# RolandFaure/Hairsplitter

Measured on AMD Instinct MI355X. Metric: aligned read-bp/sec through call_variants+separate_reads, higher is better.
Workload: dtype u8

## Files before the change

hairsplitter_amd/csrc/hs_kernels.hip:

```cpp
#include <hip/hip_runtime.h>
#include <stdint.h>
#include "hs_device.h"
#include "hs_rh8.h"

namespace hsdev {

static __device__ __forceinline__ int lane_id() { return (int)(threadIdx.x & 63u); }
static __device__ __forceinline__ int wave_id() { return __builtin_amdgcn_readfirstlane((int)(threadIdx.x >> 6)); }

static __device__ __forceinline__ unsigned long long wave_max_u64(unsigned long long v) {
#pragma unroll
    for (int d = 32; d >= 1; d >>= 1) {
        unsigned long long o = __shfl_xor(v, d, 64);
        v = o > v ? o : v;
    }
    return v;
}
static __device__ __forceinline__ int wave_scan_incl(int v) {
    v += __builtin_amdgcn_update_dpp(0, v, 0x111, 0xf, 0xf, false);
    v += __builtin_amdgcn_update_dpp(0, v, 0x112, 0xf, 0xf, false);
    v += __builtin_amdgcn_update_dpp(0, v, 0x114, 0xf, 0xf, false);
    v += __builtin_amdgcn_update_dpp(0, v, 0x118, 0xf, 0xf, false);
    v += __builtin_amdgcn_update_dpp(0, v, 0x142, 0xa, 0xf, false);
    v += __builtin_amdgcn_update_dpp(0, v, 0x143, 0xc, 0xf, false);
// ... 114 lines not shown
    const int rd = rec_read[r];
    const int64_t roff = read_off[rd];
    const int rlen = (int)(read_off[rd + 1] - roff);
    const int pos = rec_pos[r];
    const bool fwd = rec_strand[r] != 0;
    const int64_t cig0 = rec_cig_off[r], cig1 = rec_cig_off[r + 1];
    const int n_chunks = (int)((cig1 - cig0 + 63) >> 6);
    const int32_t* __restrict__ cs = chunk_start + 4 * rec_chunk_off[r];
    uint8_t* __restrict__ out = pile + pile_off[r];
    const uint8_t* __restrict__ ctgp = contig_seq + coff;
    const uint8_t* __restrict__ rdp = read_seq + roff;
    const unsigned long long lt_mask = (1ull << lane) - 1ull;
    const int rd_xor = fwd ? 0 : -1, rd_add = fwd ? 0 : rlen, rd_cmpl = fwd ? 0 : 3;

    int klo = 0, khi = n_chunks - 1;
    while (klo < khi) { const int mid = (klo + khi + 1) >> 1; if (cs[4 * mid] <= e_first) klo = mid; else khi = mid - 1; }

    int p1 = 2, p2 = 1;
    int nerr = 0, nlen = 0;
    for (int k = klo; k < n_chunks; ++k) {
        const int ev_base = cs[4 * k + 0];
        if (ev_base >= e1) break;
        const int t_cur = cs[4 * k + 1], q_cur = cs[4 * k + 2];
        const int64_t oi = cig0 + ((int64_t)k << 6) + lane;
        const bool in_range = oi < cig1;
        const uint32_t op = in_range ? cigar[oi] : 0xFu;
        const int code = in_range ? (int)(op & 15u) : 15;
        const OpAdv a = op_advances(op, in_range);
        const int ev_inc = wave_scan_incl(a.ev), rd_inc = wave_scan_incl(a.rd), rf_inc = wave_scan_incl(a.rf);
        const int ev_ex = ev_inc - a.ev;
        const int chunk_ev = __builtin_amdgcn_readlane(ev_inc, 63);
        const bool nz = a.ev > 0;
        const unsigned long long nzmask = __ballot(nz);
        wave_lds_sync();
        const bool isM = code == 0 || code == 7 || code == 8;
        s_op[wv][lane] = make_int4(ev_ex, t_cur + rd_inc - a.rd, q_cur + rf_inc - a.rf, (isM ? 1 : 0) | (code == 2 ? 3 : 0));
        if (nz) s_nzlane[wv][__popcll(nzmask & lt_mask)] = (uint8_t)lane;
        const int lo_el = e_first > ev_base ? e_first - ev_base : 0;
        const int hi_el = (e1 - ev_base) < chunk_ev ? (e1 - ev_base) : chunk_ev;
        const int lo_commit = e0 - ev_base;
        const unsigned span_commit = hi_el > lo_commit ? (unsigned)(hi_el - lo_commit) : 0u;

        uint8_t* const flags = &s_flag[wv][0][0];
        for (int eb = lo_el; eb < hi_el; eb += 64 * PU) {
#pragma unroll
            for (int z = 0; z < PU / 4; ++z) reinterpret_cast<uint32_t*>(flags)[lane + 64 * z] = 0u;
            wave_lds_sync();
            {
                const int rel = ev_ex - eb;
                if (nz && (unsigned)rel < (unsigned)(64 * PU)) flags[rel] = 1;
            }
            wave_lds_sync();
            int before = __popcll(__ballot(nz && ev_ex < eb));
            int q_[PU], c_[PU], cref_[PU];
            bool act_[PU], wr_[PU], jm_[PU];
#pragma unroll
            for (int u = 0; u < PU; ++u) {
                const int w0 = eb + 64 * u;
                const int own = (int)flags[64 * u + lane];
                const unsigned long long fm = __ballot(own != 0);
                const int e = w0 + lane;
                const int rank = (before - 1 + own + (int)__builtin_amdgcn_mbcnt_hi((uint32_t)(fm >> 32), __builtin_amdgcn_mbcnt_lo((uint32_t)fm, 0u))) & 63;
                before += __popcll(fm);
                const int4 od = s_op[wv][s_nzlane[wv][rank]];
                const int off = e - od.x;
                const bool refc = (od.w & 1) != 0, jD = (od.w & 2) != 0;
                const int t = od.y + off;
                const int q = od.z + (refc ? off : 0);
                act_[u] = (unsigned)(e - lo_commit) < span_commit && (unsigned)q < (unsigned)L;
                wr_[u] = refc; jm_[u] = od.w == 1; q_[u] = q;
                const int tt = clamp_i32(t, rlen - 1);
                const int bb = (int)rdp[(unsigned)((tt ^ rd_xor) + rd_add)];
                cref_[u] = (int)ctgp[(unsigned)clamp_i32(q, L - 1)];
                c_[u] = jD ? 4 : (bb ^ rd_cmpl);
            }
#pragma unroll
            for (int u = 0; u < PU; ++u) {
                const int w0 = eb + 64 * u;
                if (w0 >= hi_el) break;
                const int c = c_[u];
                const int cu1 = wave_shr1(c, p1);
                const int cu2 = wave_shr1(cu1, p2);
                nlen += __popcll(__ballot(act_[u]));
                nerr += __popcll(__ballot(act_[u] && !(jm_[u] && c == cref_[u])));
                if (act_[u] && wr_[u]) out[(unsigned)(q_[u] - pos)] = (uint8_t)(33 + 5 * cu2 + cu1 + 25 * c);
                const int nv = (hi_el - w0) < 64 ? (hi_el - w0) : 64;
                const int last = __builtin_amdgcn_readlane(c, nv - 1);
                const int last2 = nv >= 2 ? __builtin_amdgcn_readlane(c, nv - 2) : p1;
                p2 = last2; p1 = last;
            }
        }
    }
    if (lane == 0 && nlen > 0) {
        atomicAdd(&rec_stats[4 * r + 1], nerr);
        atomicAdd(&rec_stats[4 * r + 2], nlen);
    }
}

typedef uint32_t __attribute__((aligned(1))) u32_unaligned;
typedef uint16_t __attribute__((aligned(1))) u16_unaligned;
typedef uint32_t u32x4_unaligned __attribute__((ext_vector_type(4), aligned(1)));
static __device__ __forceinline__ uint32_t opaque(uint32_t x) { asm("" : "+v"(x)); return x; }
static __device__ __forceinline__ uint32_t bytes_ff(uint32_t x01) { return opaque(x01 << 8) - x01; }
static __device__ __forceinline__ uint32_t byte_sum(uint32_t x, uint32_t acc) { return __builtin_amdgcn_sad_u8(x, 0u, acc); }
static __device__ __forceinline__ uint32_t low_bytes(int n) { return n >= 4 ? 0xffffffffu : ((1u << (8 * n)) - 1u); }

#include "hs_kernels_runs.inc"

__global__ __launch_bounds__(256) void k_pileup_flagged_records(
    const uint8_t* __restrict__ contig_seq, const int64_t* __restrict__ contig_off,
    const uint8_t* __restrict__ read_seq, const int64_t* __restrict__ read_off,
    const int32_t* __restrict__ rec_read, const int32_t* __restrict__ rec_contig,
    const int32_t* __restrict__ rec_pos, const uint8_t* __restrict__ rec_strand,
    const int64_t* __restrict__ rec_cig_off, const uint32_t* __restrict__ cigar,
    const int64_t* __restrict__ pile_off, const int64_t* __restrict__ rec_chunk_off,
    const int32_t* __restrict__ chunk_start, int n_rec, int ev_per_task, uint8_t* __restrict__ pile, int32_t* __restrict__ rec_stats) {
    __shared__ PileupLds lds;
    const int lane = lane_id();
    const int wv = wave_id();
    const int n_waves = (int)gridDim.x * 4;
    for (int base = ((int)blockIdx.x * 4 + wv) * 64; base < n_rec; base += n_waves * 64) {
        const int rr = base + lane;
        bool flagged = false;
        if (rr < n_rec && rec_chunk_off[rr + 1] > rec_chunk_off[rr]) flagged = (chunk_start[4 * rec_chunk_off[rr] + 3] & 1) != 0;
        unsigned long long m = __ballot(flagged);
        while (m) {
            const int r = base + __builtin_ctzll(m);
            m &= m - 1ull;
            const int n_ev = rec_stats[4 * r + 3];
            for (int e0 = 0; e0 < n_ev; e0 += ev_per_task)
                pileup_task_per_event(lds, lane, wv, r, e0, ev_per_task, contig_seq, contig_off, read_seq, read_off, rec_read, rec_contig, rec_pos,
                                      rec_strand, rec_cig_off, cigar, pile_off, rec_chunk_off, chunk_start, pile, rec_stats);
        }
    }
}

#define HS_NBINS 125
#define HS_LIST_CAP 512
#ifndef HS_K2_INFLIGHT
#define HS_K2_INFLIGHT 16
#endif
template <int CB, bool FULL>
static __device__ __forceinline__ void column_stats_tail(const uint32_t* __restrict__ hw, int tid, int lane, int64_t g, int64_t total,
                                                         hs_colstat_dev* __restrict__ stats, int min_second, int32_t* __restrict__ sel_count,
                                                         int64_t* __restrict__ sel_gpos, int32_t* __restrict__ sel_depth, int sel_cap,
                                                         int64_t g_lo = 0, int64_t g_hi = 0x7fffffffffffffffll, int32_t* __restrict__ sel_ent = nullptr) {
    constexpr int PER_WORD = 4 / CB;
    constexpr int NWORDS = (HS_NBINS + PER_WORD - 1) / PER_WORD;
    int k0 = 0, k1 = 0, k2 = 0, k3 = 0;
    int c0 = 0, c1 = 0, c2 = 0, c3 = 0, c4 = 0;
    int depth = 0;
    if (!FULL) {
        if (g < total) {
            typedef unsigned short us2 __attribute__((ext_vector_type(2)));
            us2 m0a = {0, 0}, m1a = {0, 0}, m0b = {0, 0}, m1b = {0, 0};
#pragma unroll 4
            for (int w = 0; w < NWORDS; ++w) {
                const uint32_t word = hw[w * 256 + tid];
                us2 va, vb;
                if (CB == 1) {
                    depth = (int)__builtin_amdgcn_sad_u8(word, 0u, (uint32_t)depth);
                    va = __builtin_bit_cast(us2, word & 0x00ff00ffu);
                    vb = __builtin_bit_cast(us2, __builtin_amdgcn_perm(0u, word, 0x0c030c01u));
                } else {
                    depth += (int)(word & 0xffffu) + (int)(word >> 16);
                    va = __builtin_bit_cast(us2, word);
                    vb = us2{0, 0};
                }
                const us2 la = __builtin_elementwise_min(va, m0a);
                m1a = __builtin_elementwise_max(m1a, la);
                m0a = __builtin_elementwise_max(m0a, va);
                if (CB == 1) {
                    const us2 lb = __builtin_elementwise_min(vb, m0b);
                    m1b = __builtin_elementwise_max(m1b, lb);
                    m0b = __builtin_elementwise_max(m0b, vb);
                }
            }
            const int tops[8] = {m0a.x, m1a.x, m0a.y, m1a.y, m0b.x, m1b.x, m0b.y, m1b.y};
#pragma unroll
            for (int f = 0; f < 8; ++f) {
                const int v = tops[f];
                const int lo2 = v < c0 ? v : c0;
                c1 = c1 > lo2 ? c1 : lo2;
                c0 = c0 > v ? c0 : v;
            }
        }
        c2 = depth > c0 + c1 ? 1 : 0;
    } else if (g < total) {
        for (int w = 0; w < NWORDS; ++w) {
            const uint32_t word = hw[w * 256 + tid];
            if (word == 0u) continue;
#pragma unroll
            for (int f = 0; f < PER_WORD; ++f) {
                const int v = (int)((word >> (8 * CB * f)) & (CB == 1 ? 0xFFu : 0xFFFFu));
                if (v == 0) continue;
                depth += v;
                if (v > c4) {
                    const int key = w * PER_WORD + f + 33;
                    if (v > c0) { c4 = c3; c3 = c2; k3 = k2; c2 = c1; k2 = k1; c1 = c0; k1 = k0; c0 = v; k0 = key; }
                    else if (v > c1) { c4 = c3; c3 = c2; k3 = k2; c2 = c1; k2 = k1; c1 = v; k1 = key; }
                    else if (v > c2) { c4 = c3; c3 = c2; k3 = k2; c2 = v; k2 = key; }
                    else if (v > c3) { c4 = c3; c3 = v; k3 = key; }
                    else c4 = v;
                }
            }
        }
        uint4 o;
        o.x = (uint32_t)k0 | ((uint32_t)k1 << 8) | ((uint32_t)k2 << 16) | ((uint32_t)k3 << 24);
        o.y = (uint32_t)c0 | ((uint32_t)c1 << 16);
        o.z = (uint32_t)c2 | ((uint32_t)c3 << 16);
        o.w = (uint32_t)c4 | ((uint32_t)(depth > 65535 ? 65535 : depth) << 16);
        reinterpret_cast<uint4*>(stats)[g] = o;
    }
    if (sel_count) {
        __shared__ int s_wc[4], s_we[4];
        const bool sel = g < total && g >= g_lo && g < g_hi && (c1 > min_second || (c1 == min_second && c2 == 0));
        const unsigned long long m = __ballot(sel);
        const int wv = tid >> 6;
        if (lane == 0) s_wc[wv] = __popcll(m);
        if (sel_ent) { const int we = wave_sum_i32(sel ? depth : 0); if (lane == 0) s_we[wv] = we; }
        __syncthreads();
        int base = 0;
        for (int w = 0; w < wv; ++w) base += s_wc[w];
        const int64_t tile0 = (int64_t)blockIdx.x * 256;
        if (sel) {
            const int64_t slot = tile0 + base + __popcll(m & ((1ull << lane) - 1ull));
            sel_gpos[slot] = g; sel_depth[slot] = depth;
        }
        if (tid == 0) { sel_count[blockIdx.x] = s_wc[0] + s_wc[1] + s_wc[2] + s_wc[3]; if (sel_ent) sel_ent[blockIdx.x] = s_we[0] + s_we[1] + s_we[2] + s_we[3]; }
    }
}

__global__ __launch_bounds__(256) void k_selection_compact(const int32_t* __restrict__ tile_cnt, const int64_t* __restrict__ tile_base,
                                                          const int64_t* __restrict__ scratch_gpos, const int32_t* __restrict__ scratch_depth,
                                                          int64_t n_tiles, int32_t* __restrict__ out_count, int64_t* __restrict__ out_gpos,
                                                          int32_t* __restrict__ out_depth, int out_cap) {
    const int64_t t = blockIdx.x;
    const int tid = (int)threadIdx.x;
    if (t == 0 && tid == 0) *out_count = (int32_t)tile_base[n_tiles];
    if (tid < tile_cnt[t]) {
        const int64_t o = tile_base[t] + tid;
        if (o < out_cap) { out_gpos[o] = scratch_gpos[t * 256 + tid]; out_depth[o] = scratch_depth[t * 256 + tid]; }
    }
}

template <int CB, bool FULL, bool PAD>
__global__ __launch_bounds__(256) void k_column_stats_tiled(
    const uint8_t* __restrict__ pile, const int64_t* __restrict__ tile_off, const int4* __restrict__ tile_ent, int64_t total,
    hs_colstat_dev* __restrict__ stats, int min_second, int32_t* __restrict__ sel_count, int64_t* __restrict__ sel_gpos,
    int32_t* __restrict__ sel_depth, int sel_cap, int64_t tile0 ,
    int64_t g_lo, int64_t g_hi, int32_t* __restrict__ sel_ent) {
    constexpr int PER_WORD = 4 / CB;
    constexpr int NWORDS = (HS_NBINS + PER_WORD - 1) / PER_WORD;
    __shared__ __attribute__((aligned(16))) uint32_t hw[NWORDS * 256];
    const int tid = (int)threadIdx.x;
    const int lane = tid & 63;
    const int64_t tile = tile0 + (int64_t)blockIdx.x;
    const int64_t g = tile * 256 + tid;
#pragma unroll
    for (int w4 = 0; w4 < NWORDS; w4 += 4) {
        const int w = w4 + (lane >> 4);
        if (w < NWORDS) *reinterpret_cast<uint4*>(&hw[w * 256 + (tid & ~63) + (lane & 15) * 4]) = make_uint4(0u, 0u, 0u, 0u);
    }
    char* const my_col = reinterpret_cast<char*>(hw) + tid * 4;
    auto bump = [&](unsigned code, bool valid) {
        if (valid) {
            const unsigned inc = 1u << ((code & (unsigned)(PER_WORD - 1)) * (unsigned)(8 * CB));
            uint32_t* at = reinterpret_cast<uint32_t*>(my_col + ((code & ~(unsigned)(PER_WORD - 1)) << (CB == 1 ? 8 : 9)));
            __hip_atomic_fetch_add(at, inc, __ATOMIC_RELAXED, __HIP_MEMORY_SCOPE_WORKGROUP);
        }
    };
    const int64_t e0 = tile_off[tile], e1 = tile_off[tile + 1];
    for (int64_t i0 = e0; i0 < e1; i0 += 64) {
        const int nrec = (e1 - i0) < 64 ? (int)(e1 - i0) : 64;
        const int4 held = tile_ent[i0 + (lane < nrec ? lane : nrec - 1)];
        auto step = [&](int i, auto n_const) {
            constexpr int NU = decltype(n_const)::value;
            unsigned code[NU]; bool in_[NU];
#pragma unroll
            for (int u = 0; u < NU; ++u) {
                const int j = i + u;
                const int first = __builtin_amdgcn_readlane(held.x, j), len = __builtin_amdgcn_readlane(held.y, j);
                const uint32_t plo = (uint32_t)__builtin_amdgcn_readlane(held.z, j), phi = (uint32_t)__builtin_amdgcn_readlane(held.w, j);
                const uint8_t* __restrict__ base = pile + (int64_t)(((uint64_t)phi << 32) | plo);
                const bool in = (unsigned)(tid - first) < (unsigned)len;
                if (PAD) code[u] = (unsigned)base[tid] - 33u;
                else {
                    const unsigned off = (unsigned)(in ? tid : (first < 0 ? 0 : first));
                    code[u] = (unsigned)base[off] - 33u;
                }
                in_[u] = in;
            }
#pragma unroll
            for (int u = 0; u < NU; ++u) bump(code[u], in_[u] && code[u] < (unsigned)HS_NBINS);
        };
        int i = 0;
        for (; i + HS_K2_INFLIGHT <= nrec; i += HS_K2_INFLIGHT) step(i, std::integral_constant<int, HS_K2_INFLIGHT>());
        for (; i + 4 <= nrec; i += 4) step(i, std::integral_constant<int, 4>());
        for (; i < nrec; ++i) step(i, std::integral_constant<int, 1>());
    }
    column_stats_tail<CB, FULL>(hw, tid, lane, g, total, stats, min_second, sel_count, sel_gpos, sel_depth, sel_cap, g_lo, g_hi, sel_ent);
}

template <bool TOP >
static __device__ __forceinline__ void column_stats_tiled_dw_body(
    const uint8_t* __restrict__ pile, const int64_t* __restrict__ tile_off, const int4* __restrict__ tile_ent, int64_t total, int min_second,
    int32_t* __restrict__ sel_count, int64_t* __restrict__ sel_gpos, int32_t* __restrict__ sel_depth, int64_t tile0, int64_t g_lo, int64_t g_hi,
    int32_t* __restrict__ sel_ent, uint2* __restrict__ sel_info) {
    constexpr int NWORDS = (HS_NBINS + 3) / 4;
    static_assert(NWORDS == 32, "the second pass splits 32 counter words over four wavefronts");
    __shared__ __attribute__((aligned(16))) uint32_t hw[NWORDS * 256];
    __shared__ unsigned long long s_b[4];
    __shared__ int s_e[4];
    __shared__ uint8_t s_item[TOP ? 256 : 4];
    __shared__ uint32_t s_part[TOP ? 4 : 1][4][64];
    const int tid = (int)threadIdx.x;
    const int lane = tid & 63, wv = wave_id();
    const int64_t tile = tile0 + (int64_t)blockIdx.x;
#pragma unroll
    for (int x = 0; x < NWORDS * 256 / (256 * 4); ++x) reinterpret_cast<uint4*>(hw)[x * 256 + tid] = make_uint4(0u, 0u, 0u, 0u);
    __syncthreads();
    char* const my_cols = reinterpret_cast<char*>(hw) + lane * 4;
    auto bump = [&](unsigned code, bool valid, int k) {
        if (valid) {
            const unsigned inc = 1u << ((code & 3u) * 8u);
            uint32_t* at = reinterpret_cast<uint32_t*>(my_cols + 256 * k + ((code & ~3u) << 8));
#if defined(HS_K2_ABL) && HS_K2_ABL == 1
            asm volatile("" :: "v"(at), "v"(inc));
#else
            __hip_atomic_fetch_add(at, inc, __ATOMIC_RELAXED, __HIP_MEMORY_SCOPE_WORKGROUP);
#endif
        }
    };
    const int64_t e0 = tile_off[tile], e1 = tile_off[tile + 1];
    for (int64_t i0 = e0; i0 < e1; i0 += 64) {
        const int nrec = (e1 - i0) < 64 ? (int)(e1 - i0) : 64;
        const int4 held = tile_ent[i0 + (lane < nrec ? lane : nrec - 1)];
        auto step = [&](int j, auto n_const) {
            constexpr int NU = decltype(n_const)::value;
            uint32_t v[NU]; int first[NU], len[NU];
#pragma unroll
            for (int u = 0; u < NU; ++u) {
                const int jj = j + 4 * u;
                first[u] = __builtin_amdgcn_readlane(held.x, jj); len[u] = __builtin_amdgcn_readlane(held.y, jj);
                const uint32_t plo = (uint32_t)__builtin_amdgcn_readlane(held.z, jj), phi = (uint32_t)__builtin_amdgcn_readlane(held.w, jj);
                const uint8_t* __restrict__ base = pile + (int64_t)(((uint64_t)phi << 32) | plo);
#if defined(HS_K2_ABL) && HS_K2_ABL == 2
                v[u] = 0x41424344u + (uint32_t)lane + (uint32_t)(reinterpret_cast<uintptr_t>(base) & 3u);
#else
                v[u] = *reinterpret_cast<const u32_unaligned*>(base + 4 * lane);
#endif
            }
#pragma unroll
            for (int u = 0; u < NU; ++u) {
                if (first[u] == 0 && len[u] == 256) {
#pragma unroll
                    for (int k = 0; k < 4; ++k) { const unsigned code = ((v[u] >> (8 * k)) & 255u) - 33u; bump(code, code < (unsigned)HS_NBINS, k); }
                } else {
#pragma unroll
                    for (int k = 0; k < 4; ++k) {
                        const unsigned code = ((v[u] >> (8 * k)) & 255u) - 33u;
                        bump(code, (unsigned)(4 * lane + k - first[u]) < (unsigned)len[u] && code < (unsigned)HS_NBINS, k);
                    }
                }
            }
        };
        int j = wv;
        for (; j + 4 * 7 < nrec; j += 4 * 8) step(j, std::integral_constant<int, 8>());
        for (; j + 4 * 1 < nrec; j += 4 * 2) step(j, std::integral_constant<int, 2>());
        for (; j < nrec; j += 4) step(j, std::integral_constant<int, 1>());
    }
    __syncthreads();
    const int64_t g = tile * 256 + 4 * lane + wv;
    int c0 = 0, c1 = 0, depth = 0;
    bool sel;
    if (TOP) {
        uint32_t big = 0;
        if (g < total) {
#pragma unroll 8
            for (int w = 0; w < NWORDS; ++w) {
                const uint32_t word = hw[w * 256 + tid];
                const uint32_t t = word & 0xfcfcfcfcu;
                big = __builtin_amdgcn_msad_u8(t | 0x01010101u, t, big);
            }
        }
        sel = g < total && g >= g_lo && g < g_hi && (big >= 2u || min_second < 4);
    } else {
    if (g < total) {
        typedef unsigned short us2 __attribute__((ext_vector_type(2)));
        us2 m0a = {0, 0}, m1a = {0, 0}, m0b = {0, 0}, m1b = {0, 0};
#pragma unroll 4
        for (int w = 0; w < NWORDS; ++w) {
            const uint32_t word = hw[w * 256 + tid];
            depth = (int)__builtin_amdgcn_sad_u8(word, 0u, (uint32_t)depth);
            const us2 va = __builtin_bit_cast(us2, word & 0x00ff00ffu);
            const us2 vb = __builtin_bit_cast(us2, __builtin_amdgcn_perm(0u, word, 0x0c030c01u));
            const us2 la = __builtin_elementwise_min(va, m0a);
            m1a = __builtin_elementwise_max(m1a, la);
            m0a = __builtin_elementwise_max(m0a, va);
            const us2 lb = __builtin_elementwise_min(vb, m0b);
            m1b = __builtin_elementwise_max(m1b, lb);
            m0b = __builtin_elementwise_max(m0b, vb);
        }
        const int tops[8] = {m0a.x, m1a.x, m0a.y, m1a.y, m0b.x, m1b.x, m0b.y, m1b.y};
#pragma unroll
        for (int f = 0; f < 8; ++f) {
            const int v = tops[f];
            const int lo2 = v < c0 ? v : c0;
            c1 = c1 > lo2 ? c1 : lo2;
            c0 = c0 > v ? c0 : v;
        }
    }
    const bool third = depth > c0 + c1;
    sel = g < total && g >= g_lo && g < g_hi && (c1 > min_second || (c1 == min_second && !third));
    }
    const unsigned long long mine = __ballot(sel);
    const int we = wave_sum_i32(sel ? depth : 0);
    if (lane == 0) { s_b[wv] = mine; s_e[wv] = we; }
    __syncthreads();
    const unsigned long long below = (1ull << lane) - 1ull;
    int rank = 0, n_sel = 0;
#pragma unroll
    for (int k = 0; k < 4; ++k) {
        const unsigned long long bk = s_b[k];
        rank += __popcll(bk & below) + ((k < wv) ? (int)((bk >> lane) & 1ull) : 0);
        n_sel += __popcll(bk);
    }
    if (!TOP) {
        if (sel) {
            const int64_t slot = (int64_t)blockIdx.x * 256 + rank;
            sel_gpos[slot] = g; sel_depth[slot] = depth;
        }
        if (tid == 0) { sel_count[blockIdx.x] = n_sel; if (sel_ent) sel_ent[blockIdx.x] = s_e[0] + s_e[1] + s_e[2] + s_e[3]; }
        return;
    }
    if (n_sel == 0) { if (tid == 0) { sel_count[blockIdx.x] = 0; if (sel_ent) sel_ent[blockIdx.x] = 0; } return; }
    if (sel) s_item[rank] = (uint8_t)tid;
    __syncthreads();
    typedef unsigned short us2 __attribute__((ext_vector_type(2)));
    auto pk = [](uint32_t x) { return __builtin_bit_cast(us2, x); };
    auto insert3 = [](us2& t0, us2& t1, us2& t2, const us2 v) {
        const us2 lo0 = __builtin_elementwise_min(v, t0); t0 = __builtin_elementwise_max(v, t0);
        const us2 lo1 = __builtin_elementwise_min(lo0, t1); t1 = __builtin_elementwise_max(lo0, t1);
        t2 = __builtin_elementwise_max(lo1, t2);
    };
    auto merge3 = [](us2& a0, us2& a1, us2& a2, const us2 b0, const us2 b1, const us2 b2) {
        const us2 m = __builtin_elementwise_min(a0, b0), x = __builtin_elementwise_max(a1, b1), y = __builtin_elementwise_min(a1, b1);
        a0 = __builtin_elementwise_max(a0, b0);
        a1 = __builtin_elementwise_max(m, x);
        a2 = __builtin_elementwise_max(__builtin_elementwise_max(__builtin_elementwise_min(m, x), y), __builtin_elementwise_max(a2, b2));
    };
    int n_kept = 0, e_kept = 0;
    for (int r0 = 0; r0 < n_sel; r0 += 64) {
        const int item = r0 + lane;
        const uint32_t t_scan = s_item[item < n_sel ? item : 0];
        {
            const uint32_t* __restrict__ col = hw + t_scan + (unsigned)(8 * wv) * 256u;
            us2 a0 = {0, 0}, a1 = {0, 0}, a2 = {0, 0}, b0 = {0, 0}, b1 = {0, 0}, b2 = {0, 0};
            uint32_t dsum = 0;
#pragma unroll
            for (int j = 0; j < 8; ++j) {
                const uint32_t word = col[j * 256];
                dsum = __builtin_amdgcn_sad_u8(word, 0u, dsum);
                const uint32_t idw = (uint32_t)(4 * (8 * wv + j)) * 0x00010001u;
                insert3(a0, a1, a2, pk(((word & 0x00ff00ffu) << 8) | (idw | 0x00020000u)));
                insert3(b0, b1, b2, pk((word & 0xff00ff00u) | (idw | 0x00030001u)));
            }
            merge3(a0, a1, a2, b0, b1, b2);
            s_part[wv][0][lane] = __builtin_bit_cast(uint32_t, a0); s_part[wv][1][lane] = __builtin_bit_cast(uint32_t, a1); s_part[wv][2][lane] = __builtin_bit_cast(uint32_t, a2);
            s_part[wv][3][lane] = dsum;
        }
        __syncthreads();
        if (wv == 0) {
            us2 a0 = pk(s_part[0][0][lane]), a1 = pk(s_part[0][1][lane]), a2 = pk(s_part[0][2][lane]);
#pragma unroll
            for (int w = 1; w < 4; ++w) merge3(a0, a1, a2, pk(s_part[w][0][lane]), pk(s_part[w][1][lane]), pk(s_part[w][2][lane]));
            const uint32_t l0 = a0.x, l1 = a1.x, l2 = a2.x, h0 = a0.y, h1 = a1.y, h2 = a2.y;
            const uint32_t m = l0 < h0 ? l0 : h0, x = l1 > h1 ? l1 : h1, y = l1 < h1 ? l1 : h1;
            const uint32_t K0 = l0 > h0 ? l0 : h0, K1 = m > x ? m : x;
            uint32_t K2 = m < x ? m : x; K2 = K2 > y ? K2 : y; K2 = K2 > l2 ? K2 : l2; K2 = K2 > h2 ? K2 : h2;
            const int n0 = (int)(K0 >> 8), n1 = (int)(K1 >> 8), n2 = (int)(K2 >> 8);
            const int k0 = 33 + (int)(K0 & 255u), k1 = 33 + (int)(K1 & 255u);
            const bool tie = n0 == n1 || n1 == n2 || n1 == 0;
            const bool gt5 = n1 > 5 * n2;
            const bool central = k0 % 5 != k1 % 5 && ((k1 - 33) % 5 != 4 || (k1 / 5 % 5 != k0 % 5 && k1 / 25 % 5 != k0 % 5));
            const bool chosen = n1 > min_second || (n1 == min_second && n2 == 0);
            const bool keep = item < n_sel && chosen && (tie || (central && (n1 >= 5 || gt5)));
            const unsigned long long km = __ballot(keep);
            const int d = (int)(s_part[0][3][lane] + s_part[1][3][lane] + s_part[2][3][lane] + s_part[3][3][lane]);
            if (keep) {
                const int64_t slot = (int64_t)blockIdx.x * 256 + n_kept + __popcll(km & below);
                sel_gpos[slot] = tile * 256 + 4 * (int)(t_scan & 63u) + (int)(t_scan >> 6);
                sel_depth[slot] = d;
                sel_info[slot] = make_uint2((uint32_t)n0 | ((uint32_t)n1 << 16),
                                            (uint32_t)k0 | ((uint32_t)k1 << 8) | ((tie ? 32u  : 0u) | (gt5 ? 64u  : 0u)) << 16 | (uint32_t)(n2 < 63 ? n2 : 63) << 24 | 0x80000000u);
            }
            n_kept += __popcll(km);
            e_kept += wave_sum_i32(keep ? d : 0);
        }
        if (r0 + 64 < n_sel) __syncthreads();
    }
    if (tid == 0) { sel_count[blockIdx.x] = n_kept; if (sel_ent) sel_ent[blockIdx.x] = e_kept; }
}
__global__ __launch_bounds__(256) void k_column_stats_tiled_dw(
    const uint8_t* __restrict__ pile, const int64_t* __restrict__ tile_off, const int4* __restrict__ tile_ent, int64_t total, int min_second,
    int32_t* __restrict__ sel_count, int64_t* __restrict__ sel_gpos, int32_t* __restrict__ sel_depth, int64_t tile0, int64_t g_lo, int64_t g_hi,
    int32_t* __restrict__ sel_ent, uint2* __restrict__ sel_info) {
    column_stats_tiled_dw_body<true>(pile, tile_off, tile_ent, total, min_second, sel_count, sel_gpos, sel_depth, tile0, g_lo, g_hi, sel_ent, sel_info);
}

#define HS_SP_WORDS 4
#define HS_SP_READS 512
#define HS_SP_WAVES 16
#define HS_SP_THREADS (64 * HS_SP_WAVES)
__global__ __launch_bounds__(HS_SP_THREADS) void k_snp_planes(
    const int64_t* __restrict__ col_off, const int32_t* __restrict__ col_idx, const uint8_t* __restrict__ col_code,
    const uint8_t* __restrict__ snp_ref, const uint8_t* __restrict__ snp_alt, const int32_t* __restrict__ snp_contig,
    const int64_t* __restrict__ contig_snp_base, const int64_t* __restrict__ plane_off, const int32_t* __restrict__ words,
    const int32_t* __restrict__ n_reads, const int32_t* __restrict__ blk_contig, const int32_t* __restrict__ blk_word0, int n_snps,
    unsigned long long* __restrict__ alt, unsigned long long* __restrict__ ref,
    const int64_t* __restrict__ read_base , int32_t* __restrict__ rng_lo, int32_t* __restrict__ rng_hi) {
    __shared__ unsigned long long s_a[HS_SP_READS][HS_SP_WORDS], s_r[HS_SP_READS][HS_SP_WORDS];
    __shared__ unsigned int s_p[HS_SP_READS];
    const int tid = (int)threadIdx.x, lane = tid & 63, wv = tid >> 6;
    const int c = blk_contig[blockIdx.x];
    const int w0 = blk_word0[blockIdx.x];
    const int W = words[c], N = n_reads[c];
    const int nw = W - w0 < HS_SP_WORDS ? W - w0 : HS_SP_WORDS;
    const int64_t s0 = contig_snp_base[c] + 64ll * w0;
    unsigned long long* __restrict__ A = alt + plane_off[c];
    unsigned long long* __restrict__ R = ref + plane_off[c];
    for (int rb = 0; rb < N; rb += HS_SP_READS) {
        for (int x = tid; x < HS_SP_READS * HS_SP_WORDS; x += HS_SP_THREADS) { (&s_a[0][0])[x] = 0ull; (&s_r[0][0])[x] = 0ull; }
        if (read_base) for (int x = tid; x < HS_SP_READS; x += HS_SP_THREADS) s_p[x] = 0u;
        __syncthreads();
        {
            const int q_l = wv + HS_SP_WAVES * lane;
            const int64_t s_l = s0 + q_l;
            const bool v_l = lane < 256 / HS_SP_WAVES && q_l < 64 * nw && s_l < n_snps && snp_contig[s_l] == c;
            const int64_t e0_l = v_l ? col_off[s_l] : 0;
            const int n_l = v_l ? (int)(col_off[s_l + 1] - e0_l) : 0;
            const int al_l = v_l ? ((int)snp_ref[s_l] | ((int)snp_alt[s_l] << 8)) : 0;
            unsigned long long todo = __ballot(v_l);
            auto rl_e0 = [&](int l) { return ((int64_t)(unsigned)__builtin_amdgcn_readlane((int)(e0_l >> 32), l) << 32) | (unsigned)__builtin_amdgcn_readlane((int)(e0_l & 0xffffffffll), l); };
            int idx_n = 0, code_n = -1;
            if (todo) {
                const int l = __builtin_ctzll(todo);
                const int64_t e0 = rl_e0(l); const int n = __builtin_amdgcn_readlane(n_l, l);
                if (lane < n) { idx_n = col_idx[e0 + lane]; code_n = col_code[e0 + lane]; }
            }
            while (todo) {
                const int t = __builtin_ctzll(todo);
                todo &= todo - 1ull;
                const int q = wv + HS_SP_WAVES * t;
                const int64_t e0 = rl_e0(t);
                const int n = __builtin_amdgcn_readlane(n_l, t);
                const int al = __builtin_amdgcn_readlane(al_l, t);
                const int rbv = al & 255, abv = al >> 8;
                int idx = idx_n, code = code_n;
                idx_n = 0; code_n = -1;
                if (todo) {
                    const int l = __builtin_ctzll(todo);
                    const int64_t e0n = rl_e0(l); const int nn = __builtin_amdgcn_readlane(n_l, l);
                    if (lane < nn) { idx_n = col_idx[e0n + lane]; code_n = col_code[e0n + lane]; }
                }
                const unsigned long long bit = 1ull << (q & 63);
                const int wq = q >> 6;
                for (int eb = 0; eb < n; eb += 64) {
                    if (eb > 0) { idx = 0; code = -1; if (eb + lane < n) { idx = col_idx[e0 + eb + lane]; code = col_code[e0 + eb + lane]; } }
                    const int r = idx - rb;
                    if (code >= 0 && r >= 0 && r < HS_SP_READS) {
                        if (code == rbv) atomicOr(&s_r[r][wq], bit);
                        else if (code == abv) atomicOr(&s_a[r][wq], bit);
                        if (read_base && !(s_p[r] & (1u << wq))) atomicOr(&s_p[r], 1u << wq);
                    }
                }
            }
        }
        __syncthreads();
        const int nr = N - rb < HS_SP_READS ? N - rb : HS_SP_READS;
        for (int x = tid; x < nr * HS_SP_WORDS; x += HS_SP_THREADS) {
            const int r = x / HS_SP_WORDS, wq = x % HS_SP_WORDS;
            if (wq < nw) {
                const int64_t at = (int64_t)(rb + r) * W + w0 + wq;
                A[at] = s_a[r][wq]; R[at] = s_r[r][wq];
            }
        }
        if (read_base)
            for (int r = tid; r < nr; r += HS_SP_THREADS) {
                const unsigned int pm = s_p[r];
                if (pm) {
                    const int64_t at = read_base[c] + rb + r;
                    atomicMin(&rng_lo[at], w0 + __builtin_ctz(pm));
                    atomicMax(&rng_hi[at], w0 + 31 - __builtin_clz(pm));
                }
            }
        __syncthreads();
    }
}

#define SD_KW 16
__global__ __launch_bounds__(256) void k_simdiff(
    const uint64_t* __restrict__ alt, const uint64_t* __restrict__ ref, const int64_t* __restrict__ plane_off,
    const int32_t* __restrict__ n_reads, const int32_t* __restrict__ words, const int64_t* __restrict__ out_off,
    const int32_t* __restrict__ tile_contig, const int32_t* __restrict__ tile_i, const int32_t* __restrict__ tile_j,
    int32_t* __restrict__ sim, int32_t* __restrict__ diff, int es ,
    const int64_t* __restrict__ read_base , const int32_t* __restrict__ orig_of ,
    const int32_t* __restrict__ rng_lo, const int32_t* __restrict__ rng_hi) {
    __shared__ uint64_t s_planes[4][64][SD_KW + 1];
    __shared__ int s_rows[2][64];
    __shared__ int s_rng[4];
    uint64_t (*sAi)[SD_KW + 1] = s_planes[0]; uint64_t (*sRi)[SD_KW + 1] = s_planes[1];
    uint64_t (*sAj)[SD_KW + 1] = s_planes[2]; uint64_t (*sRj)[SD_KW + 1] = s_planes[3];
    const int tid = (int)threadIdx.x;
    const int c = tile_contig[blockIdx.x];
    const int i0 = tile_i[blockIdx.x] * 64, j0 = tile_j[blockIdx.x] * 64;
    const int N = n_reads[c], W = words[c];
    const uint64_t* __restrict__ A = alt + plane_off[c];
    const uint64_t* __restrict__ R = ref + plane_off[c];
    int w_begin = 0, w_end = W;
    if (orig_of) {
        const int64_t rb = read_base[c];
        if (tid < 128) {
            const int side = tid >> 6, k = (side ? j0 : i0) + (tid & 63);
            int lo = 0x7fffffff, hi = -1, rd = -1;
            if (k < N) { rd = orig_of[rb + k]; lo = rng_lo[rb + rd]; hi = rng_hi[rb + rd]; }
            s_rows[side][tid & 63] = rd;
            lo = -wave_max_i32(-lo); hi = wave_max_i32(hi);
            if ((tid & 63) == 0) { s_rng[2 * side] = lo; s_rng[2 * side + 1] = hi; }
        }
        __syncthreads();
        w_begin = s_rng[0] > s_rng[2] ? s_rng[0] : s_rng[2];
        const int e = s_rng[1] < s_rng[3] ? s_rng[1] : s_rng[3];
        w_end = e + 1;
        if (w_begin >= w_end) return;
        w_begin &= ~(SD_KW - 1);
        if (w_end > W) w_end = W;
    }
    const int ti = tid >> 4, tj = tid & 15;
    int s_acc[4][4], d_acc[4][4], u_acc[4][4];
#pragma unroll
    for (int a = 0; a < 4; ++a)
#pragma unroll
        for (int b = 0; b < 4; ++b) { s_acc[a][b] = 0; d_acc[a][b] = 0; u_acc[a][b] = 0; }

    for (int w0 = w_begin; w0 < w_end; w0 += SD_KW) {
        for (int x = tid; x < 64 * SD_KW; x += 256) {
            const int row = x / SD_KW, w = x % SD_KW;
            const int gw = w0 + w;
            const int gi = orig_of ? s_rows[0][row] : (i0 + row < N ? i0 + row : -1), gj = orig_of ? s_rows[1][row] : (j0 + row < N ? j0 + row : -1);
            const bool wi = gi >= 0 && gw < W, wj = gj >= 0 && gw < W;
            sAi[row][w] = wi ? A[(int64_t)gi * W + gw] : 0ull;
            sRi[row][w] = wi ? R[(int64_t)gi * W + gw] : 0ull;
            sAj[row][w] = wj ? A[(int64_t)gj * W + gw] : 0ull;
            sRj[row][w] = wj ? R[(int64_t)gj * W + gw] : 0ull;
        }
        __syncthreads();
#pragma unroll 4
        for (int w = 0; w < SD_KW; ++w) {
            uint64_t ai[4], ri[4], aj[4], rj[4];
#pragma unroll
            for (int a = 0; a < 4; ++a) { ai[a] = sAi[ti + 16 * a][w]; ri[a] = sRi[ti + 16 * a][w]; }
#pragma unroll
            for (int b = 0; b < 4; ++b) { aj[b] = sAj[tj + 16 * b][w]; rj[b] = sRj[tj + 16 * b][w]; }
            uint64_t ui[4], uj[4];
#pragma unroll
            for (int a = 0; a < 4; ++a) { ui[a] = ai[a] | ri[a]; uj[a] = aj[a] | rj[a]; }
#pragma unroll
            for (int a = 0; a < 4; ++a)
#pragma unroll
                for (int b = 0; b < 4; ++b) {
                    s_acc[a][b] += __popcll(ai[a] & aj[b]);
                    d_acc[a][b] += __popcll(ri[a] & rj[b]);
                    u_acc[a][b] += __popcll(ui[a] & uj[b]);
                }
        }
        __syncthreads();
    }
#pragma unroll
    for (int a = 0; a < 4; ++a)
#pragma unroll
        for (int b = 0; b < 4; ++b) {
            const int paa = s_acc[a][b], prr = d_acc[a][b], puu = u_acc[a][b];
            s_acc[a][b] = 3 * paa + prr; d_acc[a][b] = puu - paa - prr;
        }
    int32_t* __restrict__ S = sim + out_off[c] * es;
    int32_t* __restrict__ D = diff + out_off[c] * es;
#pragma unroll
    for (int a = 0; a < 4; ++a)
#pragma unroll
        for (int b = 0; b < 4; ++b) {
            const int gi = i0 + ti + 16 * a, gj = j0 + tj + 16 * b;
            if (gi < N && gj < N) {
                const bool dg = gi == gj;
                S[((int64_t)gi * N + gj) * es] = dg ? 0 : s_acc[a][b];
                D[((int64_t)gi * N + gj) * es] = dg ? 0 : d_acc[a][b];
            }
        }
    if (i0 != j0) {
        int32_t* tile = reinterpret_cast<int32_t*>(&s_planes[0][0][0]);
#pragma unroll
        for (int which = 0; which < 2; ++which) {
            __syncthreads();
#pragma unroll
            for (int a = 0; a < 4; ++a)
#pragma unroll
                for (int b = 0; b < 4; ++b) tile[(tj + 16 * b) * 65 + (ti + 16 * a)] = which == 0 ? s_acc[a][b] : d_acc[a][b];
            __syncthreads();
            int32_t* __restrict__ O = which == 0 ? S : D;
            for (int x = tid; x < 64 * 64; x += 256) {
                const int rj = x >> 6, ci = x & 63;
                const int gj = j0 + rj, gi = i0 + ci;
                if (gj < N && gi < N) O[((int64_t)gj * N + gi) * es] = tile[rj * 65 + ci];
            }
        }
    }
}

__global__ __launch_bounds__(256) void k_simdiff_windows(
    const uint64_t* __restrict__ alt, const uint64_t* __restrict__ ref, const int64_t* __restrict__ plane_off, const int32_t* __restrict__ words,
    const int32_t* __restrict__ win_contig, const int64_t* __restrict__ win_mask_off, const int32_t* __restrict__ mask_ids,
    const int64_t* __restrict__ win_mat_off, const int32_t* __restrict__ tile_win, const int32_t* __restrict__ tile_i, const int32_t* __restrict__ tile_j,
    int32_t* __restrict__ wsim, int32_t* __restrict__ wdiff, int es) {
    __shared__ uint64_t s_planes[4][64][SD_KW + 1];
    uint64_t (*sAi)[SD_KW + 1] = s_planes[0]; uint64_t (*sRi)[SD_KW + 1] = s_planes[1];
    uint64_t (*sAj)[SD_KW + 1] = s_planes[2]; uint64_t (*sRj)[SD_KW + 1] = s_planes[3];
    const int tid = (int)threadIdx.x;
    const int w = tile_win[blockIdx.x];
    const int c = win_contig[w];
    const int i0 = tile_i[blockIdx.x] * 64, j0 = tile_j[blockIdx.x] * 64;
    const int64_t m0 = win_mask_off[w];
    const int m = (int)(win_mask_off[w + 1] - m0);
    const int32_t* __restrict__ ids = mask_ids + m0;
    const int W = words[c];
    const uint64_t* __restrict__ A = alt + plane_off[c];
    const uint64_t* __restrict__ R = ref + plane_off[c];
    const int ti = tid >> 4, tj = tid & 15;
    int s_acc[4][4], d_acc[4][4], u_acc[4][4];
#pragma unroll
    for (int a = 0; a < 4; ++a)
#pragma unroll
        for (int b = 0; b < 4; ++b) { s_acc[a][b] = 0; d_acc[a][b] = 0; u_acc[a][b] = 0; }
    for (int w0 = 0; w0 < W; w0 += SD_KW) {
        for (int x = tid; x < 64 * SD_KW; x += 256) {
            const int row = x / SD_KW, ww = x % SD_KW;
            const int gw = w0 + ww;
            const bool wi = i0 + row < m && gw < W, wj = j0 + row < m && gw < W;
            const int64_t ri = wi ? ids[i0 + row] : 0, rj = wj ? ids[j0 + row] : 0;
            sAi[row][ww] = wi ? A[ri * W + gw] : 0ull;
            sRi[row][ww] = wi ? R[ri * W + gw] : 0ull;
            sAj[row][ww] = wj ? A[rj * W + gw] : 0ull;
            sRj[row][ww] = wj ? R[rj * W + gw] : 0ull;
        }
        __syncthreads();
#pragma unroll 4
        for (int ww = 0; ww < SD_KW; ++ww) {
            uint64_t ai[4], ri[4], aj[4], rj[4];
#pragma unroll
            for (int a = 0; a < 4; ++a) { ai[a] = sAi[ti + 16 * a][ww]; ri[a] = sRi[ti + 16 * a][ww]; }
#pragma unroll
            for (int b = 0; b < 4; ++b) { aj[b] = sAj[tj + 16 * b][ww]; rj[b] = sRj[tj + 16 * b][ww]; }
            uint64_t ui[4], uj[4];
#pragma unroll
            for (int a = 0; a < 4; ++a) { ui[a] = ai[a] | ri[a]; uj[a] = aj[a] | rj[a]; }
#pragma unroll
            for (int a = 0; a < 4; ++a)
#pragma unroll
                for (int b = 0; b < 4; ++b) {
                    s_acc[a][b] += __popcll(ai[a] & aj[b]);
                    d_acc[a][b] += __popcll(ri[a] & rj[b]);
                    u_acc[a][b] += __popcll(ui[a] & uj[b]);
                }
        }
        __syncthreads();
    }
#pragma unroll
    for (int a = 0; a < 4; ++a)
#pragma unroll
        for (int b = 0; b < 4; ++b) {
            const int paa = s_acc[a][b], prr = d_acc[a][b], puu = u_acc[a][b];
            s_acc[a][b] = 3 * paa + prr; d_acc[a][b] = puu - paa - prr;
        }
    int32_t* __restrict__ S = wsim + win_mat_off[w] * es;
    int32_t* __restrict__ D = wdiff + win_mat_off[w] * es;
#pragma unroll
    for (int a = 0; a < 4; ++a)
#pragma unroll
        for (int b = 0; b < 4; ++b) {
            const int gi = i0 + ti + 16 * a, gj = j0 + tj + 16 * b;
            if (gi < m && gj < m) { S[((int64_t)gi * m + gj) * es] = s_acc[a][b]; D[((int64_t)gi * m + gj) * es] = d_acc[a][b]; }
        }
}

struct Table2x2 { int n00, n01, n10, n11; };

static __device__ __forceinline__ float chi_square_dev(const Table2x2& d) {
    const int n = d.n00 + d.n01 + d.n10 + d.n11;
    if (n == 0) return 0;
    const float pmax1 = float(d.n10 + d.n11) / n;
    const float pmax2 = float(d.n01 + d.n11) / n;
    if (pmax1 * (1 - pmax1) == 0 && pmax2 * (1 - pmax2) == 0) return -1;
    if (pmax1 * pmax2 * (1 - pmax1) * (1 - pmax2) == 0) return 0;
    const float e00 = (1 - pmax1) * (1 - pmax2) * n, e01 = (1 - pmax1) * pmax2 * n;
// ... 680 lines not shown
```

Measured before the change: 126.6 billion.

## Split column top-3 scan into per-lane slices merged with DPP instead of LDS

The second pass of the tiled column-stats kernel used to have each of four wavefronts scan 8 counter words for 64 items, write partials to LDS, and let wave 0 merge and emit. Now each item is split across a quad (or pair of quads) of lanes. Each lane scans a slice of words and the top-3 and depth are merged through DPP lane swizzles, so all four waves process distinct items in parallel. Kept counts are combined via a small per-wave ballot table with double-buffered parity. This removes the LDS partial buffer, most barriers and wave-0 serialisation, at the cost of more lanes idle per item and a different slot-ordering scheme.

```diff
diff --git a/hairsplitter_amd/csrc/hs_kernels.hip b/hairsplitter_amd/csrc/hs_kernels.hip
--- a/hairsplitter_amd/csrc/hs_kernels.hip
+++ b/hairsplitter_amd/csrc/hs_kernels.hip
@@ -440,6 +440,9 @@
     column_stats_tail<CB, FULL>(hw, tid, lane, g, total, stats, min_second, sel_count, sel_gpos, sel_depth, sel_cap, g_lo, g_hi, sel_ent);
 }
 
+#ifndef HS_K2_SLICES
+#define HS_K2_SLICES 4
+#endif
 template <bool TOP >
 static __device__ __forceinline__ void column_stats_tiled_dw_body(
     const uint8_t* __restrict__ pile, const int64_t* __restrict__ tile_off, const int4* __restrict__ tile_ent, int64_t total, int min_second,
@@ -451,7 +454,8 @@
     __shared__ unsigned long long s_b[4];
     __shared__ int s_e[4];
     __shared__ uint8_t s_item[TOP ? 256 : 4];
-    __shared__ uint32_t s_part[TOP ? 4 : 1][4][64];
+    __shared__ unsigned long long s_kb[2][4];
+    __shared__ int s_ke[2][4];
     const int tid = (int)threadIdx.x;
     const int lane = tid & 63, wv = wave_id();
     const int64_t tile = tile0 + (int64_t)blockIdx.x;
@@ -588,55 +592,78 @@
         a1 = __builtin_elementwise_max(m, x);
         a2 = __builtin_elementwise_max(__builtin_elementwise_max(__builtin_elementwise_min(m, x), y), __builtin_elementwise_max(a2, b2));
     };
+    constexpr int SL = HS_K2_SLICES, IPW = 64 / SL, WPS = NWORDS / SL;
+    static_assert(SL == 4 || SL == 8, "the slices of an item are merged inside a quad, or inside two neighbouring quads");
+    const int slice = lane & (SL - 1);
+    const uint32_t code0 = (uint32_t)(4 * WPS * slice) * 0x00010001u;
     int n_kept = 0, e_kept = 0;
-    for (int r0 = 0; r0 < n_sel; r0 += 64) {
-        const int item = r0 + lane;
-        const uint32_t t_scan = s_item[item < n_sel ? item : 0];
-        {
-            const uint32_t* __restrict__ col = hw + t_scan + (unsigned)(8 * wv) * 256u;
+    for (int r0 = 0, par = 0; r0 < n_sel; r0 += 4 * IPW, par ^= 1) {
+        const int item = r0 + IPW * wv + lane / SL;
+        const bool solo = n_sel - r0 <= IPW;
+        bool keep = false;
+        unsigned long long km = 0ull;
+        int d = 0, we = 0, n0 = 0, n1 = 0, n2 = 0, k0 = 0, k1 = 0;
+        bool tie = false, gt5 = false;
+        uint32_t t_scan = 0;
+        if (r0 + IPW * wv < n_sel) {
+            t_scan = s_item[item < n_sel ? item : 0];
+            const uint32_t* __restrict__ col = hw + t_scan + (unsigned)(WPS * slice) * 256u;
             us2 a0 = {0, 0}, a1 = {0, 0}, a2 = {0, 0}, b0 = {0, 0}, b1 = {0, 0}, b2 = {0, 0};
             uint32_t dsum = 0;
 #pragma unroll
-            for (int j = 0; j < 8; ++j) {
+            for (int j = 0; j < WPS; ++j) {
                 const uint32_t word = col[j * 256];
                 dsum = __builtin_amdgcn_sad_u8(word, 0u, dsum);
-                const uint32_t idw = (uint32_t)(4 * (8 * wv + j)) * 0x00010001u;
+                const uint32_t idw = (uint32_t)(4 * j) * 0x00010001u;
                 insert3(a0, a1, a2, pk(((word & 0x00ff00ffu) << 8) | (idw | 0x00020000u)));
                 insert3(b0, b1, b2, pk((word & 0xff00ff00u) | (idw | 0x00030001u)));
             }
             merge3(a0, a1, a2, b0, b1, b2);
-            s_part[wv][0][lane] = __builtin_bit_cast(uint32_t, a0); s_part[wv][1][lane] = __builtin_bit_cast(uint32_t, a1); s_part[wv][2][lane] = __builtin_bit_cast(uint32_t, a2);
-            s_part[wv][3][lane] = dsum;
-        }
-        __syncthreads();
-        if (wv == 0) {
-            us2 a0 = pk(s_part[0][0][lane]), a1 = pk(s_part[0][1][lane]), a2 = pk(s_part[0][2][lane]);
-#pragma unroll
-            for (int w = 1; w < 4; ++w) merge3(a0, a1, a2, pk(s_part[w][0][lane]), pk(s_part[w][1][lane]), pk(s_part[w][2][lane]));
+            a0 = pk(__builtin_bit_cast(uint32_t, a0) + code0); a1 = pk(__builtin_bit_cast(uint32_t, a1) + code0); a2 = pk(__builtin_bit_cast(uint32_t, a2) + code0);
+#define HS_K2_MERGE_DPP(CTRL) { \
+                const us2 o0 = pk((uint32_t)__builtin_amdgcn_update_dpp(0, (int)__builtin_bit_cast(uint32_t, a0), CTRL, 0xf, 0xf, false)); \
+                const us2 o1 = pk((uint32_t)__builtin_amdgcn_update_dpp(0, (int)__builtin_bit_cast(uint32_t, a1), CTRL, 0xf, 0xf, false)); \
+                const us2 o2 = pk((uint32_t)__builtin_amdgcn_update_dpp(0, (int)__builtin_bit_cast(uint32_t, a2), CTRL, 0xf, 0xf, false)); \
+                merge3(a0, a1, a2, o0, o1, o2); \
+                dsum += (uint32_t)__builtin_amdgcn_update_dpp(0, (int)dsum, CTRL, 0xf, 0xf, false); }
+            HS_K2_MERGE_DPP(0xB1)
+            HS_K2_MERGE_DPP(0x4E)
+            if (SL == 8) HS_K2_MERGE_DPP(0x141)
+#undef HS_K2_MERGE_DPP
             const uint32_t l0 = a0.x, l1 = a1.x, l2 = a2.x, h0 = a0.y, h1 = a1.y, h2 = a2.y;
             const uint32_t m = l0 < h0 ? l0 : h0, x = l1 > h1 ? l1 : h1, y = l1 < h1 ? l1 : h1;
             const uint32_t K0 = l0 > h0 ? l0 : h0, K1 = m > x ? m : x;
             uint32_t K2 = m < x ? m : x; K2 = K2 > y ? K2 : y; K2 = K2 > l2 ? K2 : l2; K2 = K2 > h2 ? K2 : h2;
-            const int n0 = (int)(K0 >> 8), n1 = (int)(K1 >> 8), n2 = (int)(K2 >> 8);
-            const int k0 = 33 + (int)(K0 & 255u), k1 = 33 + (int)(K1 & 255u);
-            const bool tie = n0 == n1 || n1 == n2 || n1 == 0;
-            const bool gt5 = n1 > 5 * n2;
+            n0 = (int)(K0 >> 8); n1 = (int)(K1 >> 8); n2 = (int)(K2 >> 8);
+            k0 = 33 + (int)(K0 & 255u); k1 = 33 + (int)(K1 & 255u);
+            tie = n0 == n1 || n1 == n2 || n1 == 0;
+            gt5 = n1 > 5 * n2;
             const bool central = k0 % 5 != k1 % 5 && ((k1 - 33) % 5 != 4 || (k1 / 5 % 5 != k0 % 5 && k1 / 25 % 5 != k0 % 5));
             const bool chosen = n1 > min_second || (n1 == min_second && n2 == 0);
-            const bool keep = item < n_sel && chosen && (tie || (central && (n1 >= 5 || gt5)));
-            const unsigned long long km = __ballot(keep);
-            const int d = (int)(s_part[0][3][lane] + s_part[1][3][lane] + s_part[2][3][lane] + s_part[3][3][lane]);
-            if (keep) {
-                const int64_t slot = (int64_t)blockIdx.x * 256 + n_kept + __popcll(km & below);
-                sel_gpos[slot] = tile * 256 + 4 * (int)(t_scan & 63u) + (int)(t_scan >> 6);
-                sel_depth[slot] = d;
-                sel_info[slot] = make_uint2((uint32_t)n0 | ((uint32_t)n1 << 16),
-                                            (uint32_t)k0 | ((uint32_t)k1 << 8) | ((tie ? 32u  : 0u) | (gt5 ? 64u  : 0u)) << 16 | (uint32_t)(n2 < 63 ? n2 : 63) << 24 | 0x80000000u);
-            }
-            n_kept += __popcll(km);
-            e_kept += wave_sum_i32(keep ? d : 0);
-        }
-        if (r0 + 64 < n_sel) __syncthreads();
+            keep = item < n_sel && slice == 0 && chosen && (tie || (central && (n1 >= 5 || gt5)));
+            km = __ballot(keep);
+            d = (int)dsum;
+            if (sel_ent) we = wave_sum_i32(keep ? d : 0);
+        }
+        int base = n_kept;
+        if (solo) { n_kept += __popcll(km); e_kept += we; }
+        else {
+            if (lane == 0) { s_kb[par][wv] = km; s_ke[par][wv] = we; }
+            __syncthreads();
+#pragma unroll
+            for (int k = 0; k < 4; ++k) {
+                const int c = __popcll(s_kb[par][k]);
+                base += k < wv ? c : 0;
+                n_kept += c; e_kept += s_ke[par][k];
+            }
+        }
+        if (keep) {
+            const int64_t slot = (int64_t)blockIdx.x * 256 + base + __popcll(km & below);
+            sel_gpos[slot] = tile * 256 + 4 * (int)(t_scan & 63u) + (int)(t_scan >> 6);
+            sel_depth[slot] = d;
+            sel_info[slot] = make_uint2((uint32_t)n0 | ((uint32_t)n1 << 16),
+                                        (uint32_t)k0 | ((uint32_t)k1 << 8) | ((tie ? 32u  : 0u) | (gt5 ? 64u  : 0u)) << 16 | (uint32_t)(n2 < 63 ? n2 : 63) << 24 | 0x80000000u);
+        }
     }
     if (tid == 0) { sel_count[blockIdx.x] = n_kept; if (sel_ent) sel_ent[blockIdx.x] = e_kept; }
 }
```

Result: no change. 128.6 billion (median of 5 runs) (+1.5%).
